# nicolas1805961/Cardiac-Segmentation-Optical-flow

Measured on AMD Instinct MI355X. Metric: cine frames/sec (seg+flow) at 256x256, higher is better.
Workload: dtype f16 MFMA hi/lo split, f32 accumulate (f32-class); 1 GPU; BASELINE config 4: joint seg+flow over 256x256x30 cine slices; Generic_UNet(32 base, 6 pools) 4-flip TTA on every frame + SegFlowGaussian(video.yaml) two-chunk ED-anchored recurrence + fused label warp; image=256x256

## Files before the change

cardiac-segmentation-optical-flow_amd/csrc/conv_wino.hip:

```cpp
#include <hip/hip_fp16.h>
#include <stdlib.h>

#include "conv.h"
#include "profile.h"

namespace cf {
namespace {

typedef float f32x16 __attribute__((ext_vector_type(16)));
typedef float f32x4v __attribute__((ext_vector_type(4)));
typedef unsigned u32x2 __attribute__((ext_vector_type(2)));
typedef unsigned u32x4 __attribute__((ext_vector_type(4)));
typedef _Float16 f16x8 __attribute__((ext_vector_type(8)));
typedef _Float16 f16x4 __attribute__((ext_vector_type(4)));

struct WinoGeom {
    int TW, UW, RT, TH, PH, QW;
    int LINE, ROWP;
    int tiles_x, tiles_y;
    int nchunk, c1_pad;
    int ntask;
};

constexpr int W_REC = 80, W_CK = 16, W_NSTEP = 12;
constexpr int PS_NBUF = 4;
CF_CLOCK_DECL(g_clock_wino)
#ifdef CF_CLOCK_STAMPS
__device__ unsigned long long g_wino_phase[12];
#define WINO_T() __builtin_amdgcn_s_memtime()
#define WINO_ADD(i, v) do { if (lane == 0 && (wave == 0 || wave == 4)) atomicAdd(&g_wino_phase[i], (unsigned long long)(v)); } while (0)
#else
#define WINO_T() 0ULL
#define WINO_ADD(i, v) do { } while (0)
#endif

__device__ __forceinline__ void split_f16(float x, _Float16& hi, _Float16& lo) {
    hi = (_Float16)x;
    lo = (_Float16)(x - (float)hi);
}

__device__ __forceinline__ float from_lane_below(float v) {
    const int i = __builtin_bit_cast(int, v);
    return __builtin_bit_cast(float, __builtin_amdgcn_update_dpp(i, i, 0x111, 0xf, 0xf, false));
}
__device__ __forceinline__ float from_lane_above(float v) {
    const int i = __builtin_bit_cast(int, v);
    return __builtin_bit_cast(float, __builtin_amdgcn_update_dpp(i, i, 0x101, 0xf, 0xf, false));
}

template <int NTW>
__device__ __forceinline__ void wino_activate(f32x16 (&acc)[4][NTW], int act) {
#define CF_WINO_ACT_LOOP(A)                                                     \
    _Pragma("unroll") for (int e = 0; e < 2; ++e)                               \
    _Pragma("unroll") for (int nt = 0; nt < NTW; ++nt)                          \
    _Pragma("unroll") for (int r = 0; r < 16; ++r) {                            \
        acc[e][nt][r] = act_apply(acc[e][nt][r], A);                            \
        __builtin_amdgcn_sched_barrier(0);  \
    }
    switch (act) {
        case CF_ACT_GELU: CF_WINO_ACT_LOOP(CF_ACT_GELU) break;
        case CF_ACT_RELU: CF_WINO_ACT_LOOP(CF_ACT_RELU) break;
        case CF_ACT_LRELU: CF_WINO_ACT_LOOP(CF_ACT_LRELU) break;
        case CF_ACT_TANH: CF_WINO_ACT_LOOP(CF_ACT_TANH) break;
        case CF_ACT_SIGMOID: CF_WINO_ACT_LOOP(CF_ACT_SIGMOID) break;
        default: break;
    }
#undef CF_WINO_ACT_LOOP
}

template <int NTW, int PRE>
__global__ void __launch_bounds__(256, NTW == 4 ? 1 : 2)
conv_wino_kernel(const ConvParams p, const WinoGeom g, const _Float16* __restrict__ wpk) {
    constexpr int REC = W_REC, CK = W_CK, NSTEP = W_NSTEP;
    constexpr int VT = NTW == 4 ? 2 : 1;
    constexpr unsigned OOB = 0x80000000u;
    extern __shared__ __attribute__((aligned(16))) unsigned char lds[];
    CF_CLOCK_BEGIN();

    const int tid = threadIdx.x;
    const int lane = tid & 63, wave = __builtin_amdgcn_readfirstlane(tid >> 6);
    const int half = lane >> 5, l31 = lane & 31;
    const int mt = blockIdx.y * 4 + wave;

    int bid = blockIdx.x;
    {
        const int nb = gridDim.x;
        const int xcd = bid & 7, qn = nb >> 3, rn = nb & 7;
        bid = ((xcd < rn) ? xcd * (qn + 1) : rn * (qn + 1) + (xcd - rn) * qn) + (bid >> 3);
    }
    const int tx = bid % g.tiles_x;
    const int t2 = bid / g.tiles_x;
    const int ty = t2 % g.tiles_y;
    const int b = t2 / g.tiles_y;
    const int x0 = tx * g.TW, y0 = ty * g.TH;
    const int HW = p.H * p.W;
    const unsigned HW4 = (unsigned)HW * 4u;
    const int buf_bytes = g.PH * g.ROWP;
    const bool do_stats = p.gn_ws != nullptr;

    const __amdgpu_buffer_rsrc_t rsrc1 =
        __builtin_amdgcn_make_buffer_rsrc(const_cast<float*>(p.x1 + (long)b * p.C1 * HW), 0, (int)((long)p.C1 * HW * 4), 0x00020000);
    const __amdgpu_buffer_rsrc_t rsrc2 = __builtin_amdgcn_make_buffer_rsrc(
        const_cast<float*>(p.x2 ? p.x2 + (long)b * p.C2 * HW : p.x1), 0, p.x2 ? (int)((long)p.C2 * HW * 4) : 0, 0x00020000);
    unsigned v_off[VT], e_off[VT], v_c4[VT];
    int v_lds[VT];
    bool v_has[VT], v_first[VT], v_last[VT];
#pragma unroll
    for (int t = 0; t < VT; ++t) {
        const int task = tid + t * 256;
        v_has[t] = task < g.ntask;
        const int q = task % g.QW;
        const int r = task / g.QW;
        const int cg = r & 3, py = r >> 2;
        const int iy = y0 - 1 + py;
        const bool row_ok = v_has[t] && (unsigned)iy < (unsigned)p.H;
        v_first[t] = q == 0;
        v_last[t] = q == g.QW - 1;
        v_off[t] = row_ok ? (unsigned)(iy * p.W + x0 + 4 * q) * 4u : OOB;
        const int ecol = v_first[t] ? x0 - 1 : x0 + g.TW;
        e_off[t] = (row_ok && (v_first[t] || v_last[t]) && (unsigned)ecol < (unsigned)p.W) ? (unsigned)(iy * p.W + ecol) * 4u : OOB;
        v_c4[t] = (unsigned)cg * 4u;
        v_lds[t] = py * g.ROWP + 2 * q * REC + cg * 8;
    }

    auto issue_loads = [&](int chunk, f32x4v (&stg)[VT][4], float (&edg)[VT][4]) {
        const int c0 = chunk * CK;
        const bool in1 = c0 < g.c1_pad;
        const unsigned cb = (unsigned)(in1 ? c0 : c0 - g.c1_pad);
        const unsigned clim = (unsigned)(in1 ? p.C1 : p.C2);
#pragma unroll
        for (int t = 0; t < VT; ++t) {
#pragma unroll
            for (int j = 0; j < 4; ++j) {
                const unsigned ch = cb + v_c4[t] + (unsigned)j;
                const bool ok = ch < clim;
                const unsigned off = ok ? v_off[t] + ch * HW4 : OOB;
                const unsigned eo = ok ? e_off[t] + ch * HW4 : OOB;
                if (in1) {
                    stg[t][j] = __builtin_bit_cast(f32x4v, __builtin_amdgcn_raw_buffer_load_b128(rsrc1, off, 0, 0));
                    edg[t][j] = __builtin_bit_cast(float, __builtin_amdgcn_raw_buffer_load_b32(rsrc1, eo, 0, 0));
                } else {
                    stg[t][j] = __builtin_bit_cast(f32x4v, __builtin_amdgcn_raw_buffer_load_b128(rsrc2, off, 0, 0));
                    edg[t][j] = __builtin_bit_cast(float, __builtin_amdgcn_raw_buffer_load_b32(rsrc2, eo, 0, 0));
                }
            }
        }
    };

    const float* ctab = reinterpret_cast<const float*>(lds + 2 * buf_bytes);
    const int ctab_n = g.nchunk * CK;
    auto pre_apply = [&](float v, float cm, float ca, float cs, bool valid) -> float {
        v = (v - cm) * ca + cs;
        v = p.in_slope < 0.f ? gelu_as(v) : (v > 0.f ? v : v * p.in_slope);
        return valid ? v : 0.f;
    };
    auto write_stage = [&](int chunk, const f32x4v (&stg)[VT][4], const float (&edg)[VT][4]) {
#pragma unroll
        for (int t = 0; t < VT; ++t) {
            unsigned char* base = lds + (chunk & 1) * buf_bytes + v_lds[t];
            f32x4v cm = {0.f, 0.f, 0.f, 0.f}, ca = cm, cs = cm;
            if (PRE) {
                const int c0 = chunk * CK + (int)v_c4[t];
                cm = *reinterpret_cast<const f32x4v*>(ctab + c0);
                ca = *reinterpret_cast<const f32x4v*>(ctab + ctab_n + c0);
                cs = *reinterpret_cast<const f32x4v*>(ctab + 2 * ctab_n + c0);
            }
            const bool valid = v_off[t] != OOB, evalid = e_off[t] != OOB;
            f16x4 hi[2][4], lo[2][4];
#pragma unroll
            for (int j = 0; j < 4; ++j) {
                float c0 = stg[t][j][0], c1 = stg[t][j][1], c2 = stg[t][j][2], c3 = stg[t][j][3], e = edg[t][j];
                if (PRE) {
                    c0 = pre_apply(c0, cm[j], ca[j], cs[j], valid);
                    c1 = pre_apply(c1, cm[j], ca[j], cs[j], valid);
                    c2 = pre_apply(c2, cm[j], ca[j], cs[j], valid);
                    c3 = pre_apply(c3, cm[j], ca[j], cs[j], valid);
                    e = pre_apply(e, cm[j], ca[j], cs[j], evalid);
                }
                float left = from_lane_below(c3), right = from_lane_above(c0);
                left = v_first[t] ? e : left;
                right = v_last[t] ? e : right;
                const float va[4] = {left - c1, c0 + c1, c1 - c0, c0 - c2};
                const float vb[4] = {c1 - c3, c2 + c3, c3 - c2, c2 - right};
#pragma unroll
                for (int pos = 0; pos < 4; ++pos) {
                    _Float16 h, l;
                    split_f16(va[pos], h, l);
                    hi[0][pos][j] = h;
                    lo[0][pos][j] = l;
                    split_f16(vb[pos], h, l);
                    hi[1][pos][j] = h;
                    lo[1][pos][j] = l;
                }
            }
            if (v_has[t]) {
#pragma unroll
                for (int pos = 0; pos < 4; ++pos)
#pragma unroll
                    for (int u = 0; u < 2; ++u) {
                        *reinterpret_cast<f16x4*>(base + pos * g.LINE + u * REC) = hi[u][pos];
                        *reinterpret_cast<f16x4*>(base + pos * g.LINE + u * REC + CK * 2) = lo[u][pos];
                    }
            }
        }
    };

    f32x4v stg[VT][4];
    float edg[VT][4];
    issue_loads(0, stg, edg);

    int b_off[NTW];
#pragma unroll
    for (int nt = 0; nt < NTW; ++nt) b_off[nt] = (nt * g.RT + l31 / g.UW) * g.ROWP + (l31 % g.UW) * REC + half * 16;

    f32x16 acc[4][NTW];
#pragma unroll
    for (int pos = 0; pos < 4; ++pos)
#pragma unroll
        for (int nt = 0; nt < NTW; ++nt)
#pragma unroll
            for (int r = 0; r < 16; ++r) acc[pos][nt][r] = 0.f;

    const f16x8* wfrag = reinterpret_cast<const f16x8*>(wpk) + (long)mt * g.nchunk * (NSTEP * 2) * 64 + lane;
    constexpr int R = NTW == 2 ? 4 : 3, D = R - 1;
    f16x8 aH[R] = {}, aL[R] = {};
    auto load_a = [&](int chunk, int step, int slot) {
        const f16x8* wc = wfrag + ((long)chunk * NSTEP + step) * 2 * 64;
        aH[slot] = wc[0];
        aL[slot] = wc[64];
    };
#pragma unroll
    for (int s = 0; s < D; ++s) load_a(0, s, s % R);
    if (PRE) {
        float* ct = reinterpret_cast<float*>(lds + 2 * buf_bytes);
        for (int k = tid; k < 3 * ctab_n; k += 256) {
            const int which = k / ctab_n, c = k - which * ctab_n;
            ct[k] = c < p.C1 ? p.in_norm[((long)b * 3 + which) * p.C1 + c] : 0.f;
        }
        __syncthreads();
    }
    write_stage(0, stg, edg);
    __syncthreads();

    constexpr int BP = NTW == 2 ? 1 : 0;
    f16x8 bH[BP + 1][NTW], bL[BP + 1][NTW];
    auto load_b = [&](const unsigned char* xb, int step, int set) {
        const int toff = (step >> 2) * g.ROWP + (step & 3) * g.LINE;
#pragma unroll
        for (int nt = 0; nt < NTW; ++nt) {
            const unsigned char* rp = xb + b_off[nt] + toff;
            bH[set][nt] = *reinterpret_cast<const f16x8*>(rp);
            bL[set][nt] = *reinterpret_cast<const f16x8*>(rp + CK * 2);
        }
    };

    for (int c = 0; c < g.nchunk; ++c) {
        const bool more = c + 1 < g.nchunk;
        const int cn = more ? c + 1 : c;
        const unsigned char* xb = lds + (c & 1) * buf_bytes;
        if (BP) load_b(xb, 0, 0);
#pragma unroll
        for (int step = 0; step < NSTEP; ++step) {
            if (step + D < NSTEP) load_a(c, step + D, (step + D) % R);
            else load_a(cn, step + D - NSTEP, (step + D) % R);
            if (step == 0) issue_loads(cn, stg, edg);
            if (BP) { if (step + 1 < NSTEP) load_b(xb, step + 1, (step + 1) & 1); }
            else load_b(xb, step, 0);
            __builtin_amdgcn_sched_barrier(0);
            const int pos = step & 3;
            const int set = BP ? (step & 1) : 0;
            const f16x8 ah = aH[step % R], al = aL[step % R];
#pragma unroll
            for (int nt = 0; nt < NTW; ++nt) {
                acc[pos][nt] = __builtin_amdgcn_mfma_f32_32x32x16_f16(al, bH[set][nt], acc[pos][nt], 0, 0, 0);
                acc[pos][nt] = __builtin_amdgcn_mfma_f32_32x32x16_f16(ah, bL[set][nt], acc[pos][nt], 0, 0, 0);
                acc[pos][nt] = __builtin_amdgcn_mfma_f32_32x32x16_f16(ah, bH[set][nt], acc[pos][nt], 0, 0, 0);
            }
        }
        if (more) write_stage(c + 1, stg, edg);
        __syncthreads();
    }

#pragma unroll
    for (int nt = 0; nt < NTW; ++nt)
#pragma unroll
        for (int r = 0; r < 16; ++r) {
            const float m0 = acc[0][nt][r], m1 = acc[1][nt][r], m2 = acc[2][nt][r], m3 = acc[3][nt][r];
            acc[0][nt][r] = (m0 + m1) + m2;
            acc[1][nt][r] = (m1 - m2) - m3;
        }

    float ssum[16], ssq[16];
#pragma unroll
    for (int r = 0; r < 16; ++r) { ssum[r] = 0.f; ssq[r] = 0.f; }
#pragma unroll
    for (int r = 0; r < 16; ++r) {
        const int co = mt * 32 + (r & 3) + 8 * (r >> 2) + 4 * half;
        float bv = 0.f;
        if (p.bias && co < p.Cout) bv = p.bias[co];
#pragma unroll
        for (int nt = 0; nt < NTW; ++nt) {
            acc[0][nt][r] = p.alpha * acc[0][nt][r] + bv;
            acc[1][nt][r] = p.alpha * acc[1][nt][r] + bv;
        }
    }
    wino_activate<NTW>(acc, p.act);
    constexpr unsigned OOB_CH = 0x40000000u;
    const __amdgpu_buffer_rsrc_t rs_out = __builtin_amdgcn_make_buffer_rsrc(
        p.out + ((long)b * p.out_ctotal + p.out_coff) * (long)HW, 0, (int)((long)(p.out_ctotal - p.out_coff) * HW * 4), 0x00020000);
    unsigned o_off[NTW];
#pragma unroll
    for (int nt = 0; nt < NTW; ++nt) {
        int li = l31;
        asm volatile("" : "+v"(li));
        const int oy = y0 + nt * g.RT + li / g.UW, ox = x0 + 2 * (li % g.UW);
        o_off[nt] = (unsigned)(oy * p.W + ox) * 4u;
    }
#pragma unroll
    for (int r = 0; r < 16; ++r) {
        const int co = mt * 32 + (r & 3) + 8 * (r >> 2) + 4 * half;
        const bool co_ok = co < p.Cout;
        const unsigned ochan = co_ok ? (unsigned)co * HW4 : OOB_CH;
#pragma unroll
        for (int nt = 0; nt < NTW; ++nt) {
            float v0 = acc[0][nt][r], v1 = acc[1][nt][r];
            if (p.res) {
                if (co_ok) {
                    const float* rp = p.res + ((long)b * p.Cout + co) * HW + (o_off[nt] >> 2);
                    v0 += rp[0];
                    v1 += rp[1];
                }
            }
            u32x2 pk;
            pk[0] = __builtin_bit_cast(unsigned, v0);
            pk[1] = __builtin_bit_cast(unsigned, v1);
            __builtin_amdgcn_raw_buffer_store_b64(pk, rs_out, o_off[nt] + ochan, 0, 0);
            const float m0 = co_ok ? v0 : 0.f, m1 = co_ok ? v1 : 0.f;
            ssum[r] += m0 + m1;
            ssq[r] += m0 * m0 + m1 * m1;
        }
    }
    if (do_stats) {
        xreduce16(ssum, lane);
        xreduce16(ssq, lane);
        float* red = reinterpret_cast<float*>(lds);
        __syncthreads();
        red[tid] = 0.f;
        __syncthreads();
        if ((lane & 1) == 0) {
            const int r = ((lane >> 4) & 1) * 8 + ((lane >> 3) & 1) * 4 + ((lane >> 2) & 1) * 2 + ((lane >> 1) & 1);
            const int cl = wave * 32 + (r & 3) + 8 * (r >> 2) + 4 * half;
            atomicAdd(&red[2 * cl], ssum[0]);
            atomicAdd(&red[2 * cl + 1], ssq[0]);
        }
        __syncthreads();
        if (tid < 128) {
            const int co = blockIdx.y * 128 + tid;
            const int cpg = p.Cout / p.gn_groups;
            if (co < p.Cout && (tid == 0 || co % cpg == 0)) {
                int n = cpg - co % cpg;
                if (n > 128 - tid) n = 128 - tid;
                if (n > p.Cout - co) n = p.Cout - co;
                float s1 = 0.f, s2 = 0.f;
                for (int j = 0; j < n; ++j) { s1 += red[2 * (tid + j)]; s2 += red[2 * (tid + j) + 1]; }
                double* w = p.gn_ws + 2L * ((long)b * p.gn_groups + co / cpg);
                atomicAdd(w, (double)s1);
                atomicAdd(w + 1, (double)s2);
            }
        }
    }
    CF_CLOCK_END(g_clock_wino);
}

struct StageRegs {
    f32x4v stg[4];
    float edg[4];
    f32x4v cm, ca, cs;
    bool valid, evalid;
};

template <int PRE>
__global__ void __launch_bounds__(512, 2)
conv_wino_ps_kernel(const ConvParams p, const WinoGeom g, const _Float16* __restrict__ wpk) {
    constexpr int NTW = 2, REC = W_REC, CK = W_CK, NSTEP = W_NSTEP;
    constexpr unsigned OOB = 0x80000000u;
    extern __shared__ __attribute__((aligned(16))) unsigned char lds[];
    CF_CLOCK_BEGIN();

    const int tid = threadIdx.x;
    const int lane = tid & 63, wave = __builtin_amdgcn_readfirstlane(tid >> 6);
    const int half = lane >> 5, l31 = lane & 31;

    const int xcd = blockIdx.x & 7, wgi = blockIdx.x >> 3, nwgx = gridDim.x >> 3;
    const int ntiles = g.tiles_x * g.tiles_y * p.B;
    const int nitems = ntiles * ((p.Cout + 127) / 128);
    const int band_lo = (int)((long)nitems * xcd / 8), band_hi = (int)((long)nitems * (xcd + 1) / 8);
    if (band_lo + wgi >= band_hi) return;
    const int n_my = (band_hi - band_lo - wgi + nwgx - 1) / nwgx;
    auto decode = [&](int i, int& cb, int& b, int& y0, int& x0) {
        const int item = band_lo + wgi + i * nwgx;
        cb = item / ntiles;
        int t = item - cb * ntiles;
        const int tx = t % g.tiles_x;
        t /= g.tiles_x;
        const int ty = t % g.tiles_y;
        b = t / g.tiles_y;
        y0 = ty * g.TH;
        x0 = tx * g.TW;
    };
    const int HW = p.H * p.W;
    const unsigned HW4 = (unsigned)HW * 4u;
    const int buf_bytes = g.PH * g.ROWP;
    const int N = n_my * g.nchunk;

    if (wave >= 4) {
        constexpr int VT = 1;
        bool has[VT], first[VT], last[VT];
        unsigned c4[VT];
        int v_lds[VT], t_py[VT], t_q[VT];
#pragma unroll
        for (int t = 0; t < VT; ++t) {
            const int task = (tid - 256) + t * 256;
            has[t] = task < g.ntask;
            const int q = task % g.QW;
            const int r = task / g.QW;
            const int cg = r & 3, py = r >> 2;
            first[t] = q == 0;
            last[t] = q == g.QW - 1;
            c4[t] = (unsigned)cg * 4u;
            v_lds[t] = py * g.ROWP + 2 * q * REC + cg * 8;
            t_py[t] = py;
            t_q[t] = q;
        }

        int ld_i = 0, ld_c = 0, ld_b = 0;
        unsigned v_off[VT], e_off[VT];
        __amdgpu_buffer_rsrc_t rsrc1, rsrc2;
        auto setup = [&](int i) __attribute__((always_inline)) {
            int cb, b, y0, x0;
            decode(i, cb, b, y0, x0);
#pragma unroll
            for (int t = 0; t < VT; ++t) {
                const int iy = y0 - 1 + t_py[t];
                const bool row_ok = has[t] && (unsigned)iy < (unsigned)p.H;
                v_off[t] = row_ok ? (unsigned)(iy * p.W + x0 + 4 * t_q[t]) * 4u + c4[t] * HW4 : OOB;
                const int ecol = first[t] ? x0 - 1 : x0 + g.TW;
                e_off[t] = (row_ok && (first[t] || last[t]) && (unsigned)ecol < (unsigned)p.W) ? (unsigned)(iy * p.W + ecol) * 4u + c4[t] * HW4 : OOB;
            }
            rsrc1 = __builtin_amdgcn_make_buffer_rsrc(const_cast<float*>(p.x1 + (long)b * p.C1 * HW), 0, (int)((long)p.C1 * HW * 4), 0x00020000);
            rsrc2 = __builtin_amdgcn_make_buffer_rsrc(const_cast<float*>(p.x2 ? p.x2 + (long)b * p.C2 * HW : p.x1), 0,
                                                      p.x2 ? (int)((long)p.C2 * HW * 4) : 0, 0x00020000);
            ld_b = b;
        };
        auto issue = [&](StageRegs (&R)[VT]) __attribute__((always_inline)) {
#if defined(CF_WINO_ABLATE) && CF_WINO_ABLATE == 4
            return;
#endif
            const int c0 = ld_c * CK;
            const bool in1 = c0 < g.c1_pad;
            const unsigned cb = (unsigned)(in1 ? c0 : c0 - g.c1_pad);
#pragma unroll
            for (int t = 0; t < VT; ++t) {
#pragma unroll
                for (int j = 0; j < 4; ++j) {
                    const unsigned ch = (cb + (unsigned)j) * HW4;
                    if (in1) {
                        R[t].stg[j] = __builtin_bit_cast(f32x4v, __builtin_amdgcn_raw_buffer_load_b128(rsrc1, v_off[t] + ch, 0, 0));
                        R[t].edg[j] = __builtin_bit_cast(float, __builtin_amdgcn_raw_buffer_load_b32(rsrc1, e_off[t] + ch, 0, 0));
                    } else {
                        R[t].stg[j] = __builtin_bit_cast(f32x4v, __builtin_amdgcn_raw_buffer_load_b128(rsrc2, v_off[t] + ch, 0, 0));
                        R[t].edg[j] = __builtin_bit_cast(float, __builtin_amdgcn_raw_buffer_load_b32(rsrc2, e_off[t] + ch, 0, 0));
                    }
                }
                if (PRE) {
                    const int c = c0 + (int)c4[t];
                    const __amdgpu_buffer_rsrc_t rn = __builtin_amdgcn_make_buffer_rsrc(const_cast<float*>(p.in_norm + (long)ld_b * 3 * p.C1), 0,
                                                                                        3 * p.C1 * 4, 0x00020000);
                    const unsigned o = c < p.C1 ? (unsigned)c * 4u : OOB;
                    R[t].cm = __builtin_bit_cast(f32x4v, __builtin_amdgcn_raw_buffer_load_b128(rn, o, 0, 0));
                    R[t].ca = __builtin_bit_cast(f32x4v, __builtin_amdgcn_raw_buffer_load_b128(rn, o + (unsigned)p.C1 * 4u, 0, 0));
                    R[t].cs = __builtin_bit_cast(f32x4v, __builtin_amdgcn_raw_buffer_load_b128(rn, o + (unsigned)p.C1 * 8u, 0, 0));
                }
                R[t].valid = v_off[t] < OOB;
                R[t].evalid = e_off[t] < OOB;
            }
            if (ld_c + 1 < g.nchunk) ++ld_c;
            else if (ld_i + 1 < n_my) { ld_c = 0; ++ld_i; setup(ld_i); }
        };
        auto pre_apply = [&](float v, float cm, float ca, float cs, bool valid) -> float {
            v = (v - cm) * ca + cs;
            v = p.in_slope < 0.f ? gelu_as(v) : (v > 0.f ? v : v * p.in_slope);
            return valid ? v : 0.f;
        };
        auto write = [&](const StageRegs (&RR)[VT], int gc) __attribute__((always_inline)) {
#if defined(CF_WINO_ABLATE) && CF_WINO_ABLATE == 1
            return;
#endif
#pragma unroll
            for (int t = 0; t < VT; ++t) {
                const StageRegs& R = RR[t];
                unsigned char* base = lds + (gc & (PS_NBUF - 1)) * buf_bytes + v_lds[t];
                f16x4 hi[2][4], lo[2][4];
#pragma unroll
                for (int j = 0; j < 4; ++j) {
                    float c0 = R.stg[j][0], c1 = R.stg[j][1], c2 = R.stg[j][2], c3 = R.stg[j][3], e = R.edg[j];
                    if (PRE) {
                        c0 = pre_apply(c0, R.cm[j], R.ca[j], R.cs[j], R.valid);
                        c1 = pre_apply(c1, R.cm[j], R.ca[j], R.cs[j], R.valid);
                        c2 = pre_apply(c2, R.cm[j], R.ca[j], R.cs[j], R.valid);
                        c3 = pre_apply(c3, R.cm[j], R.ca[j], R.cs[j], R.valid);
                        e = pre_apply(e, R.cm[j], R.ca[j], R.cs[j], R.evalid);
                    }
                    float left = from_lane_below(c3), right = from_lane_above(c0);
                    left = first[t] ? e : left;
                    right = last[t] ? e : right;
                    const float va[4] = {left - c1, c0 + c1, c1 - c0, c0 - c2};
                    const float vb[4] = {c1 - c3, c2 + c3, c3 - c2, c2 - right};
#pragma unroll
                    for (int pos = 0; pos < 4; ++pos) {
                        _Float16 h, l;
                        split_f16(va[pos], h, l);
                        hi[0][pos][j] = h;
                        lo[0][pos][j] = l;
                        split_f16(vb[pos], h, l);
                        hi[1][pos][j] = h;
                        lo[1][pos][j] = l;
                    }
                }
                if (has[t]) {
#pragma unroll
                    for (int pos = 0; pos < 4; ++pos)
#pragma unroll
                        for (int u = 0; u < 2; ++u) {
                            *reinterpret_cast<f16x4*>(base + pos * g.LINE + u * REC) = hi[u][pos];
                            *reinterpret_cast<f16x4*>(base + pos * g.LINE + u * REC + CK * 2) = lo[u][pos];
                        }
                }
            }
        };
        StageRegs A[VT], B[VT];
        setup(0);
        issue(A);
        issue(B);
        unsigned long long tw = 0, ti = 0, tb = 0;
        (void)tw; (void)ti; (void)tb;
        for (int gc = 0; gc < N; gc += 2) {
            unsigned long long t0 = WINO_T();
            write(A, gc);
            unsigned long long t1 = WINO_T();
            issue(A);
            unsigned long long t2 = WINO_T();
            tw += t1 - t0; ti += t2 - t1;
            t0 = WINO_T();
            write(B, gc + 1);
            t1 = WINO_T();
            issue(B);
            t2 = WINO_T();
            __syncthreads();
            const unsigned long long t3 = WINO_T();
            tw += t1 - t0; ti += t2 - t1; tb += t3 - t2;
        }
        WINO_ADD(3, tw); WINO_ADD(4, ti); WINO_ADD(5, tb);
        return;
    }

    int b_off[NTW];
#pragma unroll
    for (int nt = 0; nt < NTW; ++nt) b_off[nt] = (nt * g.RT + l31 / g.UW) * g.ROWP + (l31 % g.UW) * REC + half * 16;
    const long mt_stride = (long)g.nchunk * (NSTEP * 2) * 64;
    const f16x8* const wbase = reinterpret_cast<const f16x8*>(wpk) + lane;
    constexpr int R = 4, D = R - 1;
    f16x8 aH[R] = {}, aL[R] = {};
    auto load_a = [&](const f16x8* wc, int slot) {
#if defined(CF_WINO_ABLATE) && CF_WINO_ABLATE == 2
        return;
#endif
        aH[slot] = wc[0];
        aL[slot] = wc[64];
    };
    f16x8 bH[2][NTW] = {}, bL[2][NTW] = {};
    auto load_b = [&](const unsigned char* xb, int step, int set) {
#if defined(CF_WINO_ABLATE) && CF_WINO_ABLATE == 3
        return;
#endif
        const int toff = (step >> 2) * g.ROWP + (step & 3) * g.LINE;
#pragma unroll
        for (int nt = 0; nt < NTW; ++nt) {
            const unsigned char* rp = xb + b_off[nt] + toff;
            bH[set][nt] = *reinterpret_cast<const f16x8*>(rp);
            bL[set][nt] = *reinterpret_cast<const f16x8*>(rp + CK * 2);
        }
    };
    f32x16 acc[4][NTW];
    int cb, b, y0, x0;
    decode(0, cb, b, y0, x0);
    const f16x8* wf = wbase + (long)(cb * 4 + wave) * mt_stride;
#pragma unroll
    for (int s = 0; s < D; ++s) load_a(wf + (long)s * 2 * 64, s % R);

    unsigned long long tm_wait = 0, tm_comp = 0, tm_epi = 0, tm_e1 = 0, tm_e2 = 0, tm_e3 = 0, tm_mark = WINO_T();
    (void)tm_wait; (void)tm_comp; (void)tm_epi; (void)tm_mark;
    int cb_n = cb, b_n = b, y0_n = y0, x0_n = x0;
    for (int i = 0; i < n_my; ++i) {
        cb = cb_n; b = b_n; y0 = y0_n; x0 = x0_n;
        const int mt = cb * 4 + wave;
        wf = wbase + (long)mt * mt_stride;
        if (i + 1 < n_my) decode(i + 1, cb_n, b_n, y0_n, x0_n);
        const f16x8* wf_next = wbase + (long)(cb_n * 4 + wave) * mt_stride;
#pragma unroll
        for (int pos = 0; pos < 4; ++pos)
#pragma unroll
            for (int nt = 0; nt < NTW; ++nt)
#pragma unroll
                for (int r = 0; r < 16; ++r) acc[pos][nt][r] = 0.f;

        for (int c = 0; c < g.nchunk; ++c) {
            const int gc = i * g.nchunk + c;
            const f16x8* wc = wf + (long)c * NSTEP * 2 * 64;
            const f16x8* wn = (c + 1 < g.nchunk) ? wc + NSTEP * 2 * 64 : wf_next;
            {
                const unsigned long long ta = WINO_T();
                if (c == 0) tm_epi += ta - tm_mark; else tm_comp += ta - tm_mark;
                if ((gc & 1) == 0) __syncthreads();
                tm_mark = WINO_T();
                tm_wait += tm_mark - ta;
            }
            const unsigned char* xb = lds + (gc & (PS_NBUF - 1)) * buf_bytes;
            load_b(xb, 0, 0);
#pragma unroll
            for (int step = 0; step < NSTEP; ++step) {
                if (step + D < NSTEP) load_a(wc + (long)(step + D) * 2 * 64, (step + D) % R);
                else load_a(wn + (long)(step + D - NSTEP) * 2 * 64, (step + D) % R);
                if (step + 1 < NSTEP) load_b(xb, step + 1, (step + 1) & 1);
                __builtin_amdgcn_sched_barrier(0);
                const int pos = step & 3;
                const int set = step & 1;
                const f16x8 ah = aH[step % R], al = aL[step % R];
#pragma unroll
                for (int nt = 0; nt < NTW; ++nt) {
                    acc[pos][nt] = __builtin_amdgcn_mfma_f32_32x32x16_f16(al, bH[set][nt], acc[pos][nt], 0, 0, 0);
                    acc[pos][nt] = __builtin_amdgcn_mfma_f32_32x32x16_f16(ah, bL[set][nt], acc[pos][nt], 0, 0, 0);
                    acc[pos][nt] = __builtin_amdgcn_mfma_f32_32x32x16_f16(ah, bH[set][nt], acc[pos][nt], 0, 0, 0);
                }
            }
        }

        {
            const unsigned long long ta = WINO_T();
            tm_comp += ta - tm_mark;
            tm_mark = ta;
        }
#pragma unroll
        for (int nt = 0; nt < NTW; ++nt)
#pragma unroll
            for (int r = 0; r < 16; ++r) {
                const float m0 = acc[0][nt][r], m1 = acc[1][nt][r], m2 = acc[2][nt][r], m3 = acc[3][nt][r];
                acc[0][nt][r] = (m0 + m1) + m2;
                acc[1][nt][r] = (m1 - m2) - m3;
            }
        float ssum[16], ssq[16];
#pragma unroll
        for (int r = 0; r < 16; ++r) {
            ssum[r] = 0.f;
            ssq[r] = 0.f;
            const int co = mt * 32 + (r & 3) + 8 * (r >> 2) + 4 * half;
            const float bv = p.bias ? p.bias[co < p.Cout ? co : p.Cout - 1] : 0.f;
#pragma unroll
            for (int nt = 0; nt < NTW; ++nt) {
                acc[0][nt][r] = p.alpha * acc[0][nt][r] + bv;
                acc[1][nt][r] = p.alpha * acc[1][nt][r] + bv;
            }
        }
        wino_activate<NTW>(acc, p.act);
        const unsigned long long te1 = WINO_T();
        constexpr unsigned OOB_CH = 0x40000000u;
        const __amdgpu_buffer_rsrc_t rs_out = __builtin_amdgcn_make_buffer_rsrc(
            p.out + ((long)b * p.out_ctotal + p.out_coff) * (long)HW, 0, (int)((long)(p.out_ctotal - p.out_coff) * HW * 4), 0x00020000);
        unsigned o_off[NTW];
#pragma unroll
        for (int nt = 0; nt < NTW; ++nt) {
            const int oy = y0 + nt * g.RT + l31 / g.UW, ox = x0 + 2 * (l31 % g.UW);
            o_off[nt] = (unsigned)(oy * p.W + ox) * 4u;
        }
        const bool odd = (lane & 1) != 0;
        const unsigned st_off = odd ? o_off[1] - 8u : o_off[0];
#pragma unroll
        for (int r = 0; r < 16; ++r) {
            const int co = mt * 32 + (r & 3) + 8 * (r >> 2) + 4 * half;
            const bool co_ok = co < p.Cout;
            const unsigned ochan = co_ok ? (unsigned)co * HW4 : OOB_CH;
            float v[NTW][2];
#pragma unroll
            for (int nt = 0; nt < NTW; ++nt) {
                float v0 = acc[0][nt][r], v1 = acc[1][nt][r];
                if (p.res) {
                    if (co_ok) {
                        const float* rp = p.res + ((long)b * p.Cout + co) * HW + (o_off[nt] >> 2);
                        v0 += rp[0];
                        v1 += rp[1];
                    }
                }
                v[nt][0] = v0;
                v[nt][1] = v1;
                const float m0 = co_ok ? v0 : 0.f, m1 = co_ok ? v1 : 0.f;
                ssum[r] += m0 + m1;
                ssq[r] += m0 * m0 + m1 * m1;
            }
            const float k0 = odd ? v[1][0] : v[0][0], k1 = odd ? v[1][1] : v[0][1];
            const int s0 = __builtin_bit_cast(int, odd ? v[0][0] : v[1][0]), s1 = __builtin_bit_cast(int, odd ? v[0][1] : v[1][1]);
            const float r0 = __builtin_bit_cast(float, __builtin_amdgcn_update_dpp(s0, s0, 0xB1, 0xf, 0xf, false));
            const float r1 = __builtin_bit_cast(float, __builtin_amdgcn_update_dpp(s1, s1, 0xB1, 0xf, 0xf, false));
            u32x4 pk;
            pk[0] = __builtin_bit_cast(unsigned, odd ? r0 : k0);
            pk[1] = __builtin_bit_cast(unsigned, odd ? r1 : k1);
            pk[2] = __builtin_bit_cast(unsigned, odd ? k0 : r0);
            pk[3] = __builtin_bit_cast(unsigned, odd ? k1 : r1);
            __builtin_amdgcn_raw_buffer_store_b128(pk, rs_out, st_off + ochan, 0, 0);
        }
        const unsigned long long te2 = WINO_T();
        tm_e1 += te1 - tm_mark;
        tm_e2 += te2 - te1;
        if (p.gn_ws) {
            xreduce16(ssum, lane);
            xreduce16(ssq, lane);
            float s1 = ssum[0], s2 = ssq[0];
            const int cpg = p.Cout / p.gn_groups;
            const int cl = ((lane >> 1) & 1) + 2 * ((lane >> 2) & 1) + 4 * half + 8 * ((lane >> 3) & 1) + 16 * ((lane >> 4) & 1);
            int k = 0;
            const bool pow2 = (cpg & (cpg - 1)) == 0;
            if (pow2 && cpg > 1) { s1 = xor_sum<2>(s1); s2 = xor_sum<2>(s2); k = 1; }
            if (pow2 && cpg > 2) { s1 = xor_sum<4>(s1); s2 = xor_sum<4>(s2); k = 2; }
            if (pow2 && cpg > 4) { s1 = xor_sum<32>(s1); s2 = xor_sum<32>(s2); k = 3; }
            if (pow2 && cpg > 8) { s1 = xor_sum<8>(s1); s2 = xor_sum<8>(s2); k = 4; }
            if (pow2 && cpg > 16) { s1 = xor_sum<16>(s1); s2 = xor_sum<16>(s2); k = 5; }
            const int span = pow2 ? (1 << k) : 1;
            const int co = mt * 32 + cl;
            if ((lane & 1) == 0 && (cl & (span - 1)) == 0 && co < p.Cout) {
                double* w = p.gn_ws + 2L * ((long)b * p.gn_groups + co / cpg);
                atomicAdd(w, (double)s1);
                atomicAdd(w + 1, (double)s2);
            }
        }
        tm_e3 += WINO_T() - te2;
    }
    tm_epi += WINO_T() - tm_mark;
    WINO_ADD(0, tm_wait); WINO_ADD(1, tm_comp); WINO_ADD(2, tm_epi); WINO_ADD(6, 1); WINO_ADD(7, N);
    WINO_ADD(8, tm_e1); WINO_ADD(9, tm_e2); WINO_ADD(10, tm_e3);
    CF_CLOCK_END(g_clock_wino);
}

int g_wino_level = -1;
int wino_level() {
    if (g_wino_level < 0) {
        const char* e = getenv("CF_CONV_WINO");
        int v = e ? atoi(e) : 1;
        if (!(v == 0 || v == 1 || v == 2 || v == 4 || v == 8)) v = 1;
        g_wino_level = v;
    }
    return g_wino_level;
}
int wino_enabled() { return wino_level() != 0; }
int wino_force_ntw() { const int v = wino_level(); return (v == 2 || v == 4) ? v : 0; }

int wino_num_cus() { return device_cu_count(); }

bool wino_geometry(const ConvParams& p, int ntw, WinoGeom& g) {
    g.TW = p.W >= 32 ? 32 : 16;
    g.UW = g.TW / 2;
    g.RT = 32 / g.UW;
    g.TH = ntw * g.RT;
    g.PH = g.TH + 2;
    g.QW = g.TW / 4;
    g.LINE = g.UW * W_REC;
    g.ROWP = 4 * g.LINE + (g.UW == 8 ? 128 : 0);
    if (p.W % g.TW != 0 || p.H % g.TH != 0) return false;
    g.tiles_x = p.W / g.TW;
    g.tiles_y = p.H / g.TH;
    g.c1_pad = p.C2 > 0 ? ((p.C1 + W_CK - 1) / W_CK) * W_CK : (1 << 30);
    g.nchunk = p.C2 > 0 ? g.c1_pad / W_CK + (p.C2 + W_CK - 1) / W_CK : (p.C1 + W_CK - 1) / W_CK;
    g.ntask = g.PH * g.QW * 4;
    return g.ntask <= 256 * (ntw == 4 ? 2 : 1);
}

size_t wino_lds_bytes(const WinoGeom& g, bool pre) { return (size_t)2 * g.PH * g.ROWP + (pre ? (size_t)3 * g.nchunk * W_CK * sizeof(float) : 0); }
size_t wino_ps_lds_bytes(const WinoGeom& g) { return (size_t)PS_NBUF * g.PH * g.ROWP; }

template <int NTW, int PRE>
int launch_wino(const ConvParams& p, const WinoGeom& g, const _Float16* wpk, hipStream_t s) {
    const size_t lds_bytes = wino_lds_bytes(g, PRE);
    if (lds_bytes > 160 * 1024) { set_error("conv_wino: LDS tile too large"); return CF_ERR_ARG; }
    auto kern = conv_wino_kernel<NTW, PRE>;
    static bool attr_set[64] = {};
    const int dev = current_device_slot();
    if (!attr_set[dev]) {
        (void)hipFuncSetAttribute(reinterpret_cast<const void*>(kern), hipFuncAttributeMaxDynamicSharedMemorySize, 160 * 1024);
        attr_set[dev] = true;
    }
    dim3 grid((unsigned)(g.tiles_x * g.tiles_y * p.B), (unsigned)((p.Cout + 127) / 128));
    dim3 block(256);
    const double flops = 2.0 * (double)p.B * p.H * p.W * p.Cout * (p.C1 + p.C2) * 9.0;
    hipEvent_t e0, e1;
    if (profile_on() && profile_events(PK_CONV_WINO, flops, &e0, &e1))
        hipExtLaunchKernelGGL(kern, grid, block, lds_bytes, s, e0, e1, 0, p, g, wpk);
    else
        hipLaunchKernelGGL(kern, grid, block, lds_bytes, s, p, g, wpk);
    hipError_t e = hipGetLastError();
    if (e != hipSuccess) { set_error(std::string("conv_wino launch failed: ") + hipGetErrorString(e)); return CF_ERR_LAUNCH; }
    return CF_OK;
}

template <int PRE>
int launch_wino_ps(const ConvParams& p, const WinoGeom& g, const _Float16* wpk, hipStream_t s) {
    const size_t lds_bytes = wino_ps_lds_bytes(g);
    if (lds_bytes > 160 * 1024) { set_error("conv_wino (persistent): LDS buffers too large"); return CF_ERR_ARG; }
    auto kern = conv_wino_ps_kernel<PRE>;
    static bool attr_set[64] = {};
    const int dev = current_device_slot();
    if (!attr_set[dev]) {
        (void)hipFuncSetAttribute(reinterpret_cast<const void*>(kern), hipFuncAttributeMaxDynamicSharedMemorySize, 160 * 1024);
        attr_set[dev] = true;
    }
    const long nitems = (long)g.tiles_x * g.tiles_y * p.B * ((p.Cout + 127) / 128);
    long nwg = wino_num_cus();
    if (nwg > ((nitems + 7) & ~7L)) nwg = (nitems + 7) & ~7L;
    dim3 grid((unsigned)nwg), block(512);
    const double flops = 2.0 * (double)p.B * p.H * p.W * p.Cout * (p.C1 + p.C2) * 9.0;
    hipEvent_t e0, e1;
    if (profile_on() && profile_events(PK_CONV_WINO, flops, &e0, &e1))
        hipExtLaunchKernelGGL(kern, grid, block, lds_bytes, s, e0, e1, 0, p, g, wpk);
    else
        hipLaunchKernelGGL(kern, grid, block, lds_bytes, s, p, g, wpk);
    hipError_t e = hipGetLastError();
    if (e != hipSuccess) { set_error(std::string("conv_wino (persistent) launch failed: ") + hipGetErrorString(e)); return CF_ERR_LAUNCH; }
    return CF_OK;
}

int wino_pick_ntw(const ConvParams& p, WinoGeom& g) {
    const int lvl = wino_level();
    const long cblocks = (p.Cout + 127) / 128;
    if ((lvl == 1 || lvl == 8) && wino_geometry(p, 2, g) && g.ntask <= 256 && wino_ps_lds_bytes(g) <= 160 * 1024 &&
        (!p.in_norm || ((p.C1 & 3) == 0 && (reinterpret_cast<uintptr_t>(p.in_norm) & 15) == 0))) {
        const long nitems = (long)g.tiles_x * g.tiles_y * p.B * cblocks;
        if (lvl == 8 || nitems >= 2L * wino_num_cus()) return 8;
    }
    if (lvl == 8) return 0;
    const int ntw = wino_force_ntw() == 4 ? 4 : 2;
    return wino_geometry(p, ntw, g) ? ntw : 0;
}

}

static int conv_wino_form(const ConvParams& p) {
    if (!wino_enabled()) return 0;
    if (conv_terms() != 3) return 0;
    if (p.KH != 3 || p.KW != 3 || p.stride != 1 || p.pad_h != 1 || p.pad_w != 1 || p.w_bstride || p.scatter2x2) return 0;
    if (!(p.Cout % 128 == 0 || (p.Cout > 128 && p.Cout % 128 >= 96))) return 0;
    if (p.W < 16 || (p.W & 15) != 0) return 0;
    if (((reinterpret_cast<uintptr_t>(p.x1) | reinterpret_cast<uintptr_t>(p.x2)) & 15) != 0) return 0;
    const long HW = (long)p.H * p.W;
    if ((long)p.C1 * HW * 4 >= (1L << 31) || (long)p.C2 * HW * 4 >= (1L << 31)) return 0;
    if ((long)p.out_ctotal * HW * 4 >= (1L << 30)) return 0;
    if (p.in_norm && (p.C2 != 0 || (reinterpret_cast<uintptr_t>(p.in_norm) & 3) != 0)) return 0;
    if (p.gn_ws && (p.gn_groups <= 0 || p.Cout % p.gn_groups != 0)) return 0;
    WinoGeom g;
    return wino_pick_ntw(p, g);
}

bool conv_wino_applicable(const ConvParams& p) { return conv_wino_form(p) != 0; }

int launch_conv_wino(const ConvParams& p, const _Float16* wpk, hipStream_t s) {
    WinoGeom g;
    const int ntw = wino_pick_ntw(p, g);
    if (!ntw) { set_error("conv_wino: layer shape not supported"); return CF_ERR_ARG; }
    if (p.gn_ws && !p.gn_prezeroed &&
        hipMemsetAsync(p.gn_ws, 0, sizeof(double) * 2 * (size_t)p.B * p.gn_groups, s) != hipSuccess) { set_error("conv_wino: memset failed"); return CF_ERR_LAUNCH; }
    if (ntw == 8) return p.in_norm ? launch_wino_ps<1>(p, g, wpk, s) : launch_wino_ps<0>(p, g, wpk, s);
    if (p.in_norm) return ntw == 4 ? launch_wino<4, 1>(p, g, wpk, s) : launch_wino<2, 1>(p, g, wpk, s);
    return ntw == 4 ? launch_wino<4, 0>(p, g, wpk, s) : launch_wino<2, 0>(p, g, wpk, s);
}

}

using namespace cf;

static void wino_params(ConvParams& p, const float* x1, int C1, const float* x2, int C2, const float* bias, const float* res, float* out,
                        int out_ctotal, int out_coff, int B, int H, int W, int Cout, int act, float alpha, double* gn_ws, int gn_groups) {
    p.x1 = x1; p.x2 = C2 ? x2 : nullptr; p.wt = nullptr; p.bias = bias; p.res = res; p.out = out; p.w_bstride = 0;
    p.C1 = C1; p.C2 = C2; p.B = B; p.H = H; p.W = W; p.Cout = Cout; p.KH = 3; p.KW = 3; p.stride = 1;
    p.pad_h = 1; p.pad_w = 1; p.Ho = H; p.Wo = W; p.out_ctotal = out_ctotal; p.out_coff = out_coff; p.act = act; p.alpha = alpha; p.scatter2x2 = 0;
    p.gn_ws = gn_ws; p.gn_groups = gn_groups < 0 ? -gn_groups : gn_groups; p.gn_prezeroed = gn_groups < 0;
}

CF_CLOCK_READER(cf_debug_clock_wino, cf::g_clock_wino)
#ifdef CF_CLOCK_STAMPS
extern "C" int cf_debug_wino_phases(unsigned long long* out12) {
    unsigned long long* out8 = out12;
    unsigned long long z[12] = {0, 0, 0, 0, 0, 0, 0, 0, 0, 0, 0, 0};
    if (hipDeviceSynchronize() != hipSuccess) return CF_ERR_LAUNCH;
    if (hipMemcpyFromSymbol(out8, HIP_SYMBOL(cf::g_wino_phase), sizeof(z)) != hipSuccess) return CF_ERR_LAUNCH;
    if (hipMemcpyToSymbol(HIP_SYMBOL(cf::g_wino_phase), z, sizeof(z)) != hipSuccess) return CF_ERR_LAUNCH;
    return CF_OK;
}
#endif

extern "C" int cf_conv_wino_enable(int level) {
    const int prev = wino_level();
    if (level == 0 || level == 1 || level == 2 || level == 4 || level == 8) g_wino_level = level;
    return prev;
}

extern "C" int cf_conv2d_wino_form(int B, int C1, int C2, int H, int W, int Cout, int prenorm) {
    if (B <= 0 || C1 <= 0 || C2 < 0 || H <= 0 || W <= 0 || Cout <= 0) return 0;
    ConvParams p;
    float* dummy = reinterpret_cast<float*>(uintptr_t(256));
    wino_params(p, dummy, C1, C2 ? dummy : nullptr, C2, nullptr, nullptr, dummy, Cout, 0, B, H, W, Cout, CF_ACT_NONE, 1.f, nullptr, 0);
    if (prenorm) { p.in_norm = dummy; p.in_slope = 0.01f; }
    return conv_wino_form(p);
}

extern "C" int cf_conv2d_wino_ok(int B, int C1, int C2, int H, int W, int Cout, int prenorm) {
    return cf_conv2d_wino_form(B, C1, C2, H, W, Cout, prenorm) != 0 ? 1 : 0;
}

extern "C" int cf_conv2d_wino(const float* x1, int C1, const float* x2, int C2, const void* wpk, const float* bias, const float* res, float* out,
                              int out_ctotal, int out_coff, int B, int H, int W, int Cout, int act, float alpha, double* gn_ws, int gn_groups,
                              void* stream) {
    CF_REQUIRE(x1 && wpk && out, "null pointer");
    CF_REQUIRE(C1 > 0 && C2 >= 0 && (C2 == 0 || x2), "bad channel split C1=%d C2=%d", C1, C2);
    CF_REQUIRE(B > 0 && H > 0 && W > 0 && Cout > 0, "bad shape B=%d H=%d W=%d Cout=%d", B, H, W, Cout);
    CF_REQUIRE(out_coff >= 0 && out_coff + Cout <= out_ctotal, "output channel slice out of range");
    CF_REQUIRE(act >= CF_ACT_NONE && act <= CF_ACT_SIGMOID, "bad activation %d", act);
    CF_REQUIRE((reinterpret_cast<uintptr_t>(wpk) & 15) == 0, "packed weights must be 16-byte aligned");
    ConvParams p;
    wino_params(p, x1, C1, x2, C2, bias, res, out, out_ctotal, out_coff, B, H, W, Cout, act, alpha, gn_ws, gn_groups);
    CF_REQUIRE(!gn_ws || (p.gn_groups > 0 && Cout % p.gn_groups == 0 && out_coff == 0 && out_ctotal == Cout), "bad GroupNorm statistics request");
    CF_REQUIRE(conv_wino_applicable(p), "layer shape outside the Winograd kernel (3x3 / stride 1 / pad 1, Cout in whole 128-channel blocks or a last block >= 96, "
                                        "W %% 16 == 0, H a multiple of the tile rows, 16-byte aligned inputs; cf_conv2d_wino_ok answers per shape)");
    return launch_conv_wino(p, reinterpret_cast<const _Float16*>(wpk), as_stream(stream));
}

extern "C" int cf_conv2d_wino_prenorm(const float* x, int C, const float* in_norm, float in_slope, const void* wpk, const float* bias, float* out,
                                      int B, int H, int W, int Cout, float alpha, double* gn_ws, int gn_groups, void* stream) {
    CF_REQUIRE(x && wpk && out && in_norm, "null pointer");
    CF_REQUIRE(B > 0 && C > 0 && H > 0 && W > 0 && Cout > 0, "bad shape B=%d C=%d H=%d W=%d Cout=%d", B, C, H, W, Cout);
    CF_REQUIRE((reinterpret_cast<uintptr_t>(wpk) & 15) == 0, "packed weights must be 16-byte aligned");
    ConvParams p;
    wino_params(p, x, C, nullptr, 0, bias, nullptr, out, Cout, 0, B, H, W, Cout, CF_ACT_NONE, alpha, gn_ws, gn_groups);
    p.in_norm = in_norm;
    p.in_slope = in_slope;
    CF_REQUIRE(!gn_ws || (p.gn_groups > 0 && Cout % p.gn_groups == 0), "bad GroupNorm statistics request");
    CF_REQUIRE(conv_wino_applicable(p), "layer shape outside the Winograd kernel (cf_conv2d_wino_ok answers per shape)");
    return launch_conv_wino(p, reinterpret_cast<const _Float16*>(wpk), as_stream(stream));
}
```

Measured before the change: 766.1 frames/s.

## Share B fragments across adjacent output rows in NTW=2 Winograd conv

For the two-row-tile variant, output rows handled by a lane are interleaved (nt + 2*row) so that adjacent rows reuse the same input-row B fragment at different kernel-row offsets. Each input row is loaded once per step and fed to both accumulators through a reordered weight schedule with a 6-slot A register ring. This cuts LDS B reads per chunk roughly in half but raises the A-prefetch depth and register use, and changes the weight-fragment indexing order.

```diff
diff --git a/cardiac-segmentation-optical-flow_amd/csrc/conv_wino.hip b/cardiac-segmentation-optical-flow_amd/csrc/conv_wino.hip
--- a/cardiac-segmentation-optical-flow_amd/csrc/conv_wino.hip
+++ b/cardiac-segmentation-optical-flow_amd/csrc/conv_wino.hip
@@ -66,6 +66,49 @@
         default: break;
     }
 #undef CF_WINO_ACT_LOOP
+}
+
+constexpr int WS_R = 6, WS_D = 4, WS_NA = 12, WS_NSTEP = 16;
+__device__ __forceinline__ void wino_load_a(f16x8 (&aH)[WS_R], f16x8 (&aL)[WS_R], const f16x8* wc, const f16x8* wn, int a) {
+#if defined(CF_WINO_ABLATE) && CF_WINO_ABLATE == 2
+    return;
+#endif
+    const f16x8* w = a < WS_NA ? wc : wn;
+    const int an = a % WS_NA;
+    w += ((an % 3) * 4 + an / 3) * 2 * 64;
+    aH[a % WS_R] = w[0];
+    aL[a % WS_R] = w[64];
+}
+__device__ __forceinline__ void wino_load_b(f16x8 (&bH)[2], f16x8 (&bL)[2], const unsigned char* xv, int ROWP, int LINE, int step) {
+#if defined(CF_WINO_ABLATE) && CF_WINO_ABLATE == 3
+    return;
+#endif
+    const unsigned char* rp = xv + (step & 3) * ROWP + (step >> 2) * LINE;
+    bH[step & 1] = *reinterpret_cast<const f16x8*>(rp);
+    bL[step & 1] = *reinterpret_cast<const f16x8*>(rp + W_CK * 2);
+}
+template <class Hook>
+__device__ __forceinline__ void wino_chunk_shared(f32x16 (&acc)[4][2], f16x8 (&aH)[WS_R], f16x8 (&aL)[WS_R], f16x8 (&bH)[2], f16x8 (&bL)[2],
+                                                  const unsigned char* xv, int ROWP, int LINE, const f16x8* wc, const f16x8* wn, Hook&& at_step0) {
+    wino_load_b(bH, bL, xv, ROWP, LINE, 0);
+#pragma unroll
+    for (int step = 0; step < WS_NSTEP; ++step) {
+        const int pos = step >> 2, j = step & 3;
+        if (j <= 2) wino_load_a(aH, aL, wc, wn, pos * 3 + j + WS_D);
+        if (step == 0) at_step0();
+        if (step + 1 < WS_NSTEP) wino_load_b(bH, bL, xv, ROWP, LINE, step + 1);
+        __builtin_amdgcn_sched_barrier(0);
+        const f16x8 bh = bH[step & 1], bl = bL[step & 1];
+#pragma unroll
+        for (int nt = 0; nt < 2; ++nt) {
+            const int ky = j - nt;
+            if (ky < 0 || ky > 2) continue;
+            const f16x8 ah = aH[(pos * 3 + ky) % WS_R], al = aL[(pos * 3 + ky) % WS_R];
+            acc[pos][nt] = __builtin_amdgcn_mfma_f32_32x32x16_f16(al, bh, acc[pos][nt], 0, 0, 0);
+            acc[pos][nt] = __builtin_amdgcn_mfma_f32_32x32x16_f16(ah, bl, acc[pos][nt], 0, 0, 0);
+            acc[pos][nt] = __builtin_amdgcn_mfma_f32_32x32x16_f16(ah, bh, acc[pos][nt], 0, 0, 0);
+        }
+    }
 }
 
 template <int NTW, int PRE>
@@ -209,9 +252,10 @@
     float edg[VT][4];
     issue_loads(0, stg, edg);
 
+    constexpr bool SHARE = NTW == 2;
     int b_off[NTW];
 #pragma unroll
-    for (int nt = 0; nt < NTW; ++nt) b_off[nt] = (nt * g.RT + l31 / g.UW) * g.ROWP + (l31 % g.UW) * REC + half * 16;
+    for (int nt = 0; nt < NTW; ++nt) b_off[nt] = (SHARE ? nt + NTW * (l31 / g.UW) : nt * g.RT + l31 / g.UW) * g.ROWP + (l31 % g.UW) * REC + half * 16;
 
     f32x16 acc[4][NTW];
 #pragma unroll
@@ -222,15 +266,20 @@
             for (int r = 0; r < 16; ++r) acc[pos][nt][r] = 0.f;
 
     const f16x8* wfrag = reinterpret_cast<const f16x8*>(wpk) + (long)mt * g.nchunk * (NSTEP * 2) * 64 + lane;
-    constexpr int R = NTW == 2 ? 4 : 3, D = R - 1;
+    constexpr int R = SHARE ? WS_R : 3, D = SHARE ? WS_D : R - 1;
     f16x8 aH[R] = {}, aL[R] = {};
     auto load_a = [&](int chunk, int step, int slot) {
         const f16x8* wc = wfrag + ((long)chunk * NSTEP + step) * 2 * 64;
         aH[slot] = wc[0];
         aL[slot] = wc[64];
     };
-#pragma unroll
-    for (int s = 0; s < D; ++s) load_a(0, s, s % R);
+    if constexpr (SHARE) {
+#pragma unroll
+        for (int a = 0; a < D; ++a) { wino_load_a(aH, aL, wfrag, wfrag, a); __builtin_amdgcn_sched_barrier(0); }
+    } else {
+#pragma unroll
+        for (int s = 0; s < D; ++s) load_a(0, s, s % R);
+    }
     if (PRE) {
         float* ct = reinterpret_cast<float*>(lds + 2 * buf_bytes);
         for (int k = tid; k < 3 * ctab_n; k += 256) {
@@ -242,15 +291,14 @@
     write_stage(0, stg, edg);
     __syncthreads();
 
-    constexpr int BP = NTW == 2 ? 1 : 0;
-    f16x8 bH[BP + 1][NTW], bL[BP + 1][NTW];
-    auto load_b = [&](const unsigned char* xb, int step, int set) {
+    f16x8 bH[SHARE ? 2 : NTW], bL[SHARE ? 2 : NTW];
+    auto load_b = [&](const unsigned char* xb, int step) {
         const int toff = (step >> 2) * g.ROWP + (step & 3) * g.LINE;
 #pragma unroll
         for (int nt = 0; nt < NTW; ++nt) {
             const unsigned char* rp = xb + b_off[nt] + toff;
-            bH[set][nt] = *reinterpret_cast<const f16x8*>(rp);
-            bL[set][nt] = *reinterpret_cast<const f16x8*>(rp + CK * 2);
+            bH[nt] = *reinterpret_cast<const f16x8*>(rp);
+            bL[nt] = *reinterpret_cast<const f16x8*>(rp + CK * 2);
         }
     };
 
@@ -258,23 +306,25 @@
         const bool more = c + 1 < g.nchunk;
         const int cn = more ? c + 1 : c;
         const unsigned char* xb = lds + (c & 1) * buf_bytes;
-        if (BP) load_b(xb, 0, 0);
-#pragma unroll
-        for (int step = 0; step < NSTEP; ++step) {
-            if (step + D < NSTEP) load_a(c, step + D, (step + D) % R);
-            else load_a(cn, step + D - NSTEP, (step + D) % R);
-            if (step == 0) issue_loads(cn, stg, edg);
-            if (BP) { if (step + 1 < NSTEP) load_b(xb, step + 1, (step + 1) & 1); }
-            else load_b(xb, step, 0);
-            __builtin_amdgcn_sched_barrier(0);
-            const int pos = step & 3;
-            const int set = BP ? (step & 1) : 0;
-            const f16x8 ah = aH[step % R], al = aL[step % R];
-#pragma unroll
-            for (int nt = 0; nt < NTW; ++nt) {
-                acc[pos][nt] = __builtin_amdgcn_mfma_f32_32x32x16_f16(al, bH[set][nt], acc[pos][nt], 0, 0, 0);
-                acc[pos][nt] = __builtin_amdgcn_mfma_f32_32x32x16_f16(ah, bL[set][nt], acc[pos][nt], 0, 0, 0);
-                acc[pos][nt] = __builtin_amdgcn_mfma_f32_32x32x16_f16(ah, bH[set][nt], acc[pos][nt], 0, 0, 0);
+        if constexpr (SHARE) {
+            wino_chunk_shared(acc, aH, aL, bH, bL, xb + b_off[0], g.ROWP, g.LINE, wfrag + (long)c * NSTEP * 2 * 64, wfrag + (long)cn * NSTEP * 2 * 64,
+                              [&]() { issue_loads(cn, stg, edg); });
+        } else {
+#pragma unroll
+            for (int step = 0; step < NSTEP; ++step) {
+                if (step + D < NSTEP) load_a(c, step + D, (step + D) % R);
+                else load_a(cn, step + D - NSTEP, (step + D) % R);
+                if (step == 0) issue_loads(cn, stg, edg);
+                load_b(xb, step);
+                __builtin_amdgcn_sched_barrier(0);
+                const int pos = step & 3;
+                const f16x8 ah = aH[step % R], al = aL[step % R];
+#pragma unroll
+                for (int nt = 0; nt < NTW; ++nt) {
+                    acc[pos][nt] = __builtin_amdgcn_mfma_f32_32x32x16_f16(al, bH[nt], acc[pos][nt], 0, 0, 0);
+                    acc[pos][nt] = __builtin_amdgcn_mfma_f32_32x32x16_f16(ah, bL[nt], acc[pos][nt], 0, 0, 0);
+                    acc[pos][nt] = __builtin_amdgcn_mfma_f32_32x32x16_f16(ah, bH[nt], acc[pos][nt], 0, 0, 0);
+                }
             }
         }
         if (more) write_stage(c + 1, stg, edg);
@@ -313,7 +363,7 @@
     for (int nt = 0; nt < NTW; ++nt) {
         int li = l31;
         asm volatile("" : "+v"(li));
-        const int oy = y0 + nt * g.RT + li / g.UW, ox = x0 + 2 * (li % g.UW);
+        const int oy = y0 + (SHARE ? nt + NTW * (li / g.UW) : nt * g.RT + li / g.UW), ox = x0 + 2 * (li % g.UW);
         o_off[nt] = (unsigned)(oy * p.W + ox) * 4u;
     }
 #pragma unroll
@@ -564,39 +614,17 @@
         return;
     }
 
-    int b_off[NTW];
-#pragma unroll
-    for (int nt = 0; nt < NTW; ++nt) b_off[nt] = (nt * g.RT + l31 / g.UW) * g.ROWP + (l31 % g.UW) * REC + half * 16;
+    const int b_base = NTW * (l31 / g.UW) * g.ROWP + (l31 % g.UW) * REC + half * 16;
     const long mt_stride = (long)g.nchunk * (NSTEP * 2) * 64;
     const f16x8* const wbase = reinterpret_cast<const f16x8*>(wpk) + lane;
-    constexpr int R = 4, D = R - 1;
-    f16x8 aH[R] = {}, aL[R] = {};
-    auto load_a = [&](const f16x8* wc, int slot) {
-#if defined(CF_WINO_ABLATE) && CF_WINO_ABLATE == 2
-        return;
-#endif
-        aH[slot] = wc[0];
-        aL[slot] = wc[64];
-    };
-    f16x8 bH[2][NTW] = {}, bL[2][NTW] = {};
-    auto load_b = [&](const unsigned char* xb, int step, int set) {
-#if defined(CF_WINO_ABLATE) && CF_WINO_ABLATE == 3
-        return;
-#endif
-        const int toff = (step >> 2) * g.ROWP + (step & 3) * g.LINE;
-#pragma unroll
-        for (int nt = 0; nt < NTW; ++nt) {
-            const unsigned char* rp = xb + b_off[nt] + toff;
-            bH[set][nt] = *reinterpret_cast<const f16x8*>(rp);
-            bL[set][nt] = *reinterpret_cast<const f16x8*>(rp + CK * 2);
-        }
-    };
+    f16x8 aH[WS_R] = {}, aL[WS_R] = {};
+    f16x8 bH[2] = {}, bL[2] = {};
     f32x16 acc[4][NTW];
     int cb, b, y0, x0;
     decode(0, cb, b, y0, x0);
     const f16x8* wf = wbase + (long)(cb * 4 + wave) * mt_stride;
 #pragma unroll
-    for (int s = 0; s < D; ++s) load_a(wf + (long)s * 2 * 64, s % R);
+    for (int a = 0; a < WS_D; ++a) { wino_load_a(aH, aL, wf, wf, a); __builtin_amdgcn_sched_barrier(0); }
 
     unsigned long long tm_wait = 0, tm_comp = 0, tm_epi = 0, tm_e1 = 0, tm_e2 = 0, tm_e3 = 0, tm_mark = WINO_T();
     (void)tm_wait; (void)tm_comp; (void)tm_epi; (void)tm_mark;
@@ -626,23 +654,7 @@
                 tm_wait += tm_mark - ta;
             }
             const unsigned char* xb = lds + (gc & (PS_NBUF - 1)) * buf_bytes;
-            load_b(xb, 0, 0);
-#pragma unroll
-            for (int step = 0; step < NSTEP; ++step) {
-                if (step + D < NSTEP) load_a(wc + (long)(step + D) * 2 * 64, (step + D) % R);
-                else load_a(wn + (long)(step + D - NSTEP) * 2 * 64, (step + D) % R);
-                if (step + 1 < NSTEP) load_b(xb, step + 1, (step + 1) & 1);
-                __builtin_amdgcn_sched_barrier(0);
-                const int pos = step & 3;
-                const int set = step & 1;
-                const f16x8 ah = aH[step % R], al = aL[step % R];
-#pragma unroll
-                for (int nt = 0; nt < NTW; ++nt) {
-                    acc[pos][nt] = __builtin_amdgcn_mfma_f32_32x32x16_f16(al, bH[set][nt], acc[pos][nt], 0, 0, 0);
-                    acc[pos][nt] = __builtin_amdgcn_mfma_f32_32x32x16_f16(ah, bL[set][nt], acc[pos][nt], 0, 0, 0);
-                    acc[pos][nt] = __builtin_amdgcn_mfma_f32_32x32x16_f16(ah, bH[set][nt], acc[pos][nt], 0, 0, 0);
-                }
-            }
+            wino_chunk_shared(acc, aH, aL, bH, bL, xb + b_base, g.ROWP, g.LINE, wc, wn, []() {});
         }
 
         {
@@ -679,7 +691,7 @@
         unsigned o_off[NTW];
 #pragma unroll
         for (int nt = 0; nt < NTW; ++nt) {
-            const int oy = y0 + nt * g.RT + l31 / g.UW, ox = x0 + 2 * (l31 % g.UW);
+            const int oy = y0 + nt + NTW * (l31 / g.UW), ox = x0 + 2 * (l31 % g.UW);
             o_off[nt] = (unsigned)(oy * p.W + ox) * 4u;
         }
         const bool odd = (lane & 1) != 0;
```

After: 773.5 frames/s (median of 6 runs). About the same (+1.0%).
